# Xinhuan-Imperial/Lattice-Boltzmann-Method-GPU

Measured on NVIDIA B200. Metric: MLUPS, higher is better.
Workload: dtype f64

## Files before the change

### lattice_boltzmann_method_gpu_b200/csrc/lbm_api.cu

```cuda
#include <algorithm>
#include <charconv>
#include <chrono>
#include <cmath>
#include <cstdarg>
#include <cstdio>
#include <cstdlib>
#include <cstring>
#include <deque>
#include <memory>
#include <fstream>
#include <iostream>
#include <new>
#include <sstream>
#include <string>
#include <thread>
#include <vector>

#include "lbm_internal.h"
#include "geo_text.h"
#include "vtk_format.h"

namespace lbm {

static thread_local std::string g_create_error;
// ... 110 lines not shown
    size_t scratch_ints = 0;
    double last_S = 0.0;
    std::vector<long long> plane_first;
    T *d_stage = nullptr;
    size_t stage_elems = 0;
    cudaStream_t st_copy = nullptr;
    cudaEvent_t ev_gathered[2] = {nullptr, nullptr}, ev_copied[2] = {nullptr, nullptr};
    long long pend_i0 = 0, pend_i1 = 0;
    bool interior_pending = false;
    T *peer_buf[2][2] = {{nullptr, nullptr}, {nullptr, nullptr}};
    long long peer_qs[2] = {0, 0}, peer_c0[2] = {0, 0}, peer_own[2] = {0, 0};
    T *d_mail[2] = {nullptr, nullptr}, *peer_mail[2] = {nullptr, nullptr};
    long long mail_ms = 0, mail_G = 0;
    bool mail_live[2] = {false, false};
    T *d_stage_out[2] = {nullptr, nullptr}, *d_stage_in[2] = {nullptr, nullptr};
    bool mail_staged[2] = {false, false};
    unsigned long long *d_sync = nullptr;
    unsigned long long *peer_sync[2] = {nullptr, nullptr};
    int64_t sync_base = 0;
    cudaEvent_t ev_face[2] = {nullptr, nullptr};
    SolverBase *inproc_nb[2] = {nullptr, nullptr};
    bool sparse = false;
    long long n_lo_stored = 0, stored_box = 0;
    long long sp_first = 0;
    long long nseg = 0;
    long long *d_cart = nullptr, *d_chunk_off = nullptr, *d_plane_seg = nullptr;
    uint32_t *d_nodec = nullptr;
    int8_t *d_labelc = nullptr;
    int32_t *d_rec = nullptr, *d_chunk_cnt = nullptr;
    std::vector<long long> seg_plane_start;
    int32_t *d_sid = nullptr;
    uint2 *d_cmeta = nullptr;
    uint32_t *d_rec_links = nullptr;
    int32_t *d_bcslot = nullptr;
    BcLink<T> *d_bclinks = nullptr;
    std::vector<long long> sid_plane_first;
    long long own_id0 = 0, own_id1 = 0;
    long long halo_id0[2] = {0, 0}, halo_n[2] = {0, 0};
    long long face_id0[2] = {0, 0}, face_n[2] = {0, 0};

    ~Solver() override {
        join_writer();
        cudaSetDevice(d.device);
        auto fr = [](void *p) {
            if (p) cudaFree(p);
        };
        fr(d_flag), fr(d_label_ext), fr(d_label), fr(d_index), fr(d_scratch), fr(d_node), fr(d_seg), fr(d_label8);
        fr(d_fa), fr(d_fb == d_fa ? nullptr : d_fb), fr(d_rho), fr(d_ux), fr(d_uy), fr(d_uz), fr(d_plane_in), fr(d_plane_out);
        fr(d_send[0]), fr(d_send[1]), fr(d_recv[0]), fr(d_recv[1]), fr(d_acc), fr(d_cnt);
        fr(d_sid), fr(d_cmeta), fr(d_rec_links), fr(d_bcslot), fr(d_bclinks);
        fr(d_stage), fr(d_wall), fr(d_wallc), fr(d_cart), fr(d_chunk_off), fr(d_nodec), fr(d_labelc), fr(d_rec), fr(d_chunk_cnt), fr(d_plane_seg);
        fr(d_mail[0]), fr(d_mail[1]), fr(d_stage_out[0]), fr(d_stage_out[1]), fr(d_stage_in[0]), fr(d_stage_in[1]);
        fr(d_sync), fr(d_chk_shadow[0]), fr(d_chk_shadow[1]), fr(d_chk_count), fr(d_pulse), fr(d_barrier);
        if (ev0) cudaEventDestroy(ev0);
        if (ev1) cudaEventDestroy(ev1);
        for (auto &e : ev_face)
            if (e) cudaEventDestroy(e);
        for (int k = 0; k < 2; k++) {
            if (ev_gathered[k]) cudaEventDestroy(ev_gathered[k]);
            if (ev_copied[k]) cudaEventDestroy(ev_copied[k]);
        }
        if (st_copy) cudaStreamDestroy(st_copy);
        if (st) cudaStreamDestroy(st);
    }

    int store_all() const { return d.case_rule == LBM_CASE_LDC ? 1 : 0; }

    std::vector<std::pair<void *, size_t>> allocs;
    template <typename U>
    int dalloc(U **p, size_t n) {
        CK(cudaMalloc((void **)p, std::max<size_t>(n, 1) * sizeof(U)));
        dev_bytes += (int64_t)(n * sizeof(U));
        allocs.emplace_back((void *)*p, n * sizeof(U));
        return 0;
    }
    template <typename U>
    void dfree(U **p) {
        if (!*p) return;
        for (auto &a : allocs)
            if (a.first == (void *)*p) {
                dev_bytes -= (int64_t)a.second;
                a = allocs.back();
                allocs.pop_back();
                break;
            }
        cudaFree((void *)*p);
        *p = nullptr;
    }
    void release_geometry_sized() {
        if (d_fb == d_fa) d_fb = nullptr;
        dfree(&d_fa), dfree(&d_fb), dfree(&d_rho), dfree(&d_ux), dfree(&d_uy), dfree(&d_uz);
        for (int sd = 0; sd < 2; sd++) dfree(&d_send[sd]), dfree(&d_recv[sd]);
        dfree(&d_cart), dfree(&d_nodec), dfree(&d_wallc), dfree(&d_labelc), dfree(&d_rec), dfree(&d_chunk_cnt);
        dfree(&d_cmeta), dfree(&d_rec_links), dfree(&d_bcslot), dfree(&d_bclinks);
        dfree(&d_chunk_off), dfree(&d_plane_seg);
        if (d_stage) cudaFree(d_stage), d_stage = nullptr, stage_elems = 0;
        d_cur = d_nxt = nullptr;
        for (int sd = 0; sd < 2; sd++) peer_buf[sd][0] = peer_buf[sd][1] = nullptr;
    }

    int setup() {
        CK(cudaSetDevice(d.device));
        CK(cudaStreamCreateWithFlags(&st, cudaStreamNonBlocking));
        CK(cudaEventCreate(&ev0));
        CK(cudaEventCreate(&ev1));
        for (auto &e : ev_face) CK(cudaEventCreateWithFlags(&e, cudaEventDisableTiming));
// ... 407 lines not shown
            CK(launch_bc_links<T>(d_nodec, d_wallc, d_cart, d_label8, box, bc, d_plane_in, d_plane_out, own_id0, own_id1, d_tot, nullptr,
                                  nullptr, st));
            CK(cudaMemcpyAsync(&total, d_tot, sizeof(int), cudaMemcpyDeviceToHost, st));
            CK(cudaStreamSynchronize(st));
            dfree(&d_bcslot), dfree(&d_bclinks);
            if (dalloc(&d_bcslot, (size_t)std::max<long long>(ns, 1)) || dalloc(&d_bclinks, (size_t)std::max(total, 1))) return LBM_ERR_NOMEM;
            CK(cudaMemsetAsync(d_tot, 0, sizeof(int), st));
            CK(launch_bc_links<T>(d_nodec, d_wallc, d_cart, d_label8, box, bc, d_plane_in, d_plane_out, own_id0, own_id1, d_tot, d_bcslot,
                                  d_bclinks, st));
            launches += 2;
        }
        qstride = (ns + 64 + 31) & ~31LL;
        if (aa && qstride >= (1LL << 31) / 3) FAIL(LBM_ERR_ARG, "slab of %lld nodes is too large for 32-bit element offsets: use more z-slabs", ns);
        if (!d_fa) {
            const size_t fsize = (size_t)qstride * Q + 64;
            if (dalloc(&d_fa, fsize)) return LBM_ERR_NOMEM;
            if (aa) d_fb = d_fa;
            else if (dalloc(&d_fb, fsize)) return LBM_ERR_NOMEM;
            if (dalloc(&d_rho, (size_t)ns) || dalloc(&d_ux, (size_t)ns) || dalloc(&d_uy, (size_t)ns) || dalloc(&d_uz, (size_t)ns))
                return LBM_ERR_NOMEM;
            for (int sd = 0; sd < 2; sd++) {
                const size_t nb = (size_t)std::max(face_n[sd], halo_n[sd]) * 5;
                if (dalloc(&d_send[sd], nb) || dalloc(&d_recv[sd], nb)) return LBM_ERR_NOMEM;
            }
        }
        InitParams<T> ip{};
        ip.fa = d_fa, ip.fb = d_fb, ip.aa = aa ? 1 : 0, ip.qstride = qstride, ip.label = d_label;
        ip.rho = d_rho, ip.ux = d_ux, ip.uy = d_uy, ip.uz = d_uz;
        ip.box = box, ip.case_rule = d.case_rule, ip.u_max = (T)d.u_max;
        for (int i = 0; i < LBM_MAX_BC; i++) ip.bc[i] = bc[i];
        ip.plane_in = d_plane_in, ip.plane_out = d_plane_out, ip.fluid_label = fluid_label;
        CK(launch_init_sparse<T>(ip, d_cart, ns, st));
        launches++;
        CK(cudaStreamSynchronize(st));
        d_cur = d_fa, d_nxt = d_fb;
        steps = 0;
        have_init = true, have_moments = false, in_step = false;
        detach_neighbours();
        return 0;
    }

    bool speculative_pull() const {
        static const char *const force = getenv("LBM_SPECULATIVE");
        return force ? atoi(force) != 0 : (nfluid * 10 >= (int64_t)(own_z1 - own_z0) * box.plane * 9);
    }
    int preload_kernels(bool resid) {
        const bool peers = lo_halo || hi_halo;
        CK(cudaSetDevice(d.device));
        if (d.math == LBM_MATH_STRICT) CK(preload_step_kernels_strict<T>(d.storage, speculative_pull(), peers, resid));
        else CK(preload_step_kernels_fast<T>(d.storage, speculative_pull(), peers, resid));
        return 0;
    }

    StepParams<T> make_params(long long c0, long long c1, double *acc) {
        StepParams<T> p{};
        p.src = d_cur, p.dst = d_nxt, p.qstride = qstride;
        p.node = d_node, p.wall = d_wall, p.seg = d_seg, p.label8 = d_label8;
        p.rho = d_rho, p.ux = d_ux, p.uy = d_uy, p.uz = d_uz;
        p.resid = acc;
        p.box = box, p.c_begin = c0, p.c_end = c1;
        p.pdl = opt_pdl && !lo_halo && !hi_halo && in_place();
        p.fluid_label = fluid_label;
        p.tau = (T)d.tau;
        p.inv_tau = T(1.0) / p.tau;
        p.om1 = T(1.0) - T(1.0) / p.tau;
        double sc = 1.0;
        if (d.pulse_amp != 0.0) sc = 1.0 + d.pulse_amp * std::sin(2.0 * M_PI * (double)steps / d.pulse_period);
        p.pulse_scale = (T)sc;
        for (int i = 0; i < LBM_MAX_BC; i++) p.bc[i] = bc[i];
        p.plane_in = d_plane_in, p.plane_out = d_plane_out;
        p.parity = (int)(steps & 1);
        p.case_rule = d.case_rule;
        p.u_init = (T)d.u_max;
#ifdef LBM_SELFCHECK
        if (chk_prepare() == 0) {
            p.chk_lo[0] = d_fa, p.chk_hi[0] = d_fa + chk_elems, p.chk_lo[1] = d_fb, p.chk_hi[1] = d_fb + chk_elems;
            p.chk_shadow[0] = d_chk_shadow[0], p.chk_shadow[1] = d_fb == d_fa ? d_chk_shadow[0] : d_chk_shadow[1];
            p.chk_count = d_chk_count, p.chk_launch = ++chk_launch_id;
        }
#endif
        p.speculative = speculative_pull();
        return p;
    }
    int launch_range(long long c0, long long c1, bool moments, bool resid, double *acc, int face_sides = 0) {
        if (c1 <= c0) return 0;
        StepParams<T> p = make_params(c0, c1, acc);
        const int which = d_nxt == d_fa ? 0 : 1;
        for (int sd = 0; sd < 2; sd++) {
            if (!(face_sides & (1 << sd)) || !peer_mail[sd]) continue;
            T *dst = peer_mail[sd] + (p.parity ? 5 * mail_ms : 0);
            if (sd == 1) p.peer_up = dst, p.peer_up_qs = mail_ms, p.peer_up_c0 = mail_G, p.peer_up_own = mail_G;
            else p.peer_dn = dst, p.peer_dn_qs = mail_ms, p.peer_dn_c0 = mail_G, p.peer_dn_own = mail_G;
            p.peer_mail = 1, p.face_c0 = c0;
            p.mail[sd] = d_mail[sd], p.mail_ms = mail_ms, p.mail_G = mail_G;
        }
        if ((face_sides & 2) && peer_buf[1][which]) {
            p.peer_up = peer_buf[1][which], p.peer_up_qs = peer_qs[1], p.peer_up_c0 = peer_c0[1], p.peer_up_own = peer_own[1];
            p.face_c0 = sparse ? face_id0[1] : c0;
        }
        if ((face_sides & 1) && peer_buf[0][which]) {
            p.peer_dn = peer_buf[0][which], p.peer_dn_qs = peer_qs[0], p.peer_dn_c0 = peer_c0[0], p.peer_dn_own = peer_own[0];
            p.face_c0 = sparse ? face_id0[0] : c0;
        }
        if (sparse) {
            SparseParams<T> sp{};
            sp.base = p, sp.rec = d_rec, sp.nodec = d_nodec, sp.wallc = d_wallc;
            {
                static const int spw_env = getenv("LBM_SPW") ? atoi(getenv("LBM_SPW")) : 0;
                sp.spw = spw_env > 0 ? spw_env : 1;
            }
            const long long zA = c0 / box.plane - (own_z0 - box.z0), zB = c1 / box.plane - (own_z0 - box.z0);
            sp.seg_begin = seg_plane_start[(size_t)zA], sp.seg_end = seg_plane_start[(size_t)zB];
            if (d.storage == LBM_STORE_SPARSE_AA) {
                sp.cartc = d_cart, sp.cmeta = d_cmeta, sp.rec_links = d_rec_links, sp.bcslot = d_bcslot, sp.bclinks = d_bclinks;
                sp.id_begin = sid_plane_first[(size_t)(c0 / box.plane)], sp.id_end = sid_plane_first[(size_t)(c1 / box.plane)];
                sp.halo_lo_n = (int)halo_n[0], sp.halo_hi0 = (int)halo_id0[1];
                sp.pdl = sp.base.pdl;
                if (sp.base.parity == 0 ? sp.id_end <= sp.id_begin : sp.seg_end <= sp.seg_begin) return 0;
                if (d.math == LBM_MATH_STRICT) CK(launch_step_sparse_aa_strict<T>(sp, moments, resid, st));
                else CK(launch_step_sparse_aa_fast<T>(sp, moments, resid, st));
                launches++;
                return 0;
            }
            if (sp.seg_end <= sp.seg_begin) return 0;
// ... 10 lines not shown
    long long plane_c(int z_global) const { return (long long)(z_global - box.z0) * box.plane; }

    T *d_pulse = nullptr;
    size_t pulse_cap = 0;
    unsigned *d_barrier = nullptr;
    int sm_count = 0;
    static constexpr int PERSIST_MAX_STEPS = 2048, PERSIST_BAR_WORDS = 64 + 32 * 64;
    int opt_persist = -1;
    int opt_pdl = 1;
    bool use_persist() {
        if (d.storage != LBM_STORE_SPARSE_AA || lo_halo || hi_halo) return false;
#ifdef LBM_SELFCHECK
        return false;
#endif
        return opt_persist > 0;
    }
    int persist_steps(int n, bool moments_last, double *S_dev) {
        if (n <= 0) return 0;
        if (!sm_count) {
            cudaDeviceProp prop;
            CK(cudaGetDeviceProperties(&prop, d.device));
            sm_count = prop.multiProcessorCount;
            CK(cudaMalloc((void **)&d_barrier, PERSIST_BAR_WORDS * sizeof(unsigned)));
        }
        const T *pulse_dev = nullptr;
        if (d.pulse_amp != 0.0) {
            std::vector<T> tab((size_t)n);
            for (int k = 0; k < n; k++) tab[(size_t)k] = (T)(1.0 + d.pulse_amp * std::sin(2.0 * M_PI * (double)(steps + k) / d.pulse_period));
            if ((size_t)n > pulse_cap) {
                if (d_pulse) cudaFree(d_pulse), d_pulse = nullptr;
                pulse_cap = (size_t)std::max(n, 256);
                CK(cudaMalloc((void **)&d_pulse, pulse_cap * sizeof(T)));
            }
            CK(cudaMemcpyAsync(d_pulse, tab.data(), (size_t)n * sizeof(T), cudaMemcpyHostToDevice, st));
            CK(cudaStreamSynchronize(st));
            pulse_dev = d_pulse;
        }
        CK(cudaMemsetAsync(d_barrier, 0, PERSIST_BAR_WORDS * sizeof(unsigned), st));
        SparseParams<T> sp{};
        sp.base = make_params(plane_c(own_z0), plane_c(own_z1), nullptr);
        sp.rec = d_rec, sp.nodec = d_nodec, sp.wallc = d_wallc, sp.spw = 1, sp.cartc = d_cart, sp.cmeta = d_cmeta, sp.rec_links = d_rec_links;
        sp.bcslot = d_bcslot, sp.bclinks = d_bclinks;
        sp.seg_begin = seg_plane_start[0], sp.seg_end = seg_plane_start[(size_t)(own_z1 - own_z0)];
        sp.id_begin = own_id0, sp.id_end = own_id1;
        sp.halo_lo_n = 0, sp.halo_hi0 = INT32_MAX;
        const int parity0 = (int)(steps & 1);
        if (d.math == LBM_MATH_STRICT) CK(launch_sparse_aa_persist_strict<T>(sp, n, parity0, moments_last ? 1 : 0, S_dev, pulse_dev, d_barrier, sm_count, st));
        else CK(launch_sparse_aa_persist_fast<T>(sp, n, parity0, moments_last ? 1 : 0, S_dev, pulse_dev, d_barrier, sm_count, st));
        launches++;
        steps += n;
        return 0;
    }

    int step(int n, float *ms) override {
        if (!have_init) FAIL(LBM_ERR_STATE, "step before initialize");
        if (lo_halo || hi_halo) FAIL(LBM_ERR_STATE, "slab handle: use lbm_step_begin / lbm_step_end");
        if (n < 0) FAIL(LBM_ERR_ARG, "negative step count");
        CK(cudaSetDevice(d.device));
        if (ms) CK(cudaEventRecord(ev0, st));
        if (use_persist()) {
            for (int done = 0; done < n; done += PERSIST_MAX_STEPS) {
                const int nb = std::min(PERSIST_MAX_STEPS, n - done);
                int r = persist_steps(nb, done + nb == n, nullptr);
                if (r) return r;
            }
        } else {
            for (int i = 0; i < n; i++) {
                int r = launch_range(plane_c(own_z0), plane_c(own_z1), i == n - 1, false, nullptr);
                if (r) return r;
                std::swap(d_cur, d_nxt);
                steps++;
            }
        }
        if (n > 0) have_moments = true;
        if (ms) {
            CK(cudaEventRecord(ev1, st));
            CK(cudaEventSynchronize(ev1));
            CK(cudaEventElapsedTime(ms, ev0, ev1));
        } else {
            CK(cudaStreamSynchronize(st));
        }
        return 0;
    }

    double *step_acc = nullptr;
    bool step_nosync = false;
    static constexpr unsigned long long SYNC_TIMEOUT_NS = 20ull * 1000000000ull;
    int step_begin(int flags) override { return step_begin_ex(flags, nullptr); }
    int step_begin_ex(int flags, double *acc) {
        if (!have_init) FAIL(LBM_ERR_STATE, "step before initialize");
        if (in_step) FAIL(LBM_ERR_STATE, "lbm_step_begin called twice");
        CK(cudaSetDevice(d.device));
        const bool mom = flags & LBM_STEP_MOMENTS, res = flags & LBM_STEP_VELSUM;
        if (in_place() && ((lo_halo && !peer_buf[0][0] && !peer_mail[0]) || (hi_halo && !peer_buf[1][0] && !peer_mail[1])))
            FAIL(LBM_ERR_STATE, "in-place storage exchanges slab faces by peer stores only: call lbm_p2p_attach first");
        step_flags = flags;
        step_acc = acc ? acc : d_acc, step_nosync = acc != nullptr;
        if (res && !acc) CK(cudaMemsetAsync(d_acc, 0, sizeof(double), st));
        const unsigned long long done = (unsigned long long)(steps - sync_base);
        if (peer_sync[0] || peer_sync[1]) {
            CK(launch_slab_wait(d_sync, peer_sync[0] ? done : 0ull, peer_sync[1] ? done : 0ull, SYNC_TIMEOUT_NS, st));
            launches++;
        }
        for (int sd = 0; sd < 2; sd++)
            if (inproc_nb[sd]) CK(cudaStreamWaitEvent(st, inproc_nb[sd]->face_event((int)((steps + 1) & 1)), 0));
        int r;
        const int zt = own_z1 - 1, zb = own_z0;
        long long i0 = plane_c(own_z0), i1 = plane_c(own_z1);
        if (hi_halo) {
            const int sides = 2 | ((lo_halo && zb == zt) ? 1 : 0);
            if ((r = launch_range(plane_c(zt), plane_c(zt + 1), mom, res, step_acc, sides))) return r;
            if (!fused(1)) {
                if (sparse) CK(launch_halo_pack_sparse<T>(d_nxt, qstride, face_id0[1], face_n[1], 1, d_send[1], face_n[1], st));
                else CK(launch_halo_pack<T>(d_nxt, qstride, box, zt - box.z0, 1, d_send[1], st));
                launches++;
            }
            i1 = plane_c(zt);
        }
        if (lo_halo && !(hi_halo && zb == zt)) {
            if ((r = launch_range(plane_c(zb), plane_c(zb + 1), mom, res, step_acc, 1))) return r;
// ... 1583 lines not shown
```

### lattice_boltzmann_method_gpu_b200/csrc/lbm_internal.h

```cpp
#pragma once
#include <cstdint>
#include <cuda_runtime.h>

#include "../../include/lbm_b200.h"

namespace lbm {

constexpr int Q = 19;
constexpr uint32_t NODE_SKIP = 1u;
constexpr uint32_t NODE_LINKS = 0x7FFFEu;
constexpr uint32_t NODE_WALLS_ONLY = 0x80000000u;
constexpr uint32_t NODE_HAS_BC = 0x40000000u;

enum : uint8_t { SEG_BULK = 0, SEG_MIXED = 1, SEG_EMPTY = 2 };

struct BcEntry {
    int kind, naxis, nsign, vaxis, source, pulsatile;
    double value, init_value;
};

struct Box {
    int nx, ny, nz;
    int px;
    int z0, z1;
// ... 140 lines not shown
template <typename T>
cudaError_t launch_reduce_fields_sparse(const T *ux, const T *uy, const T *uz, const int8_t *labelc, const long long *cart,
                                        Box box, long long i0, long long i1, int kind, int fluid_label, int case_rule,
                                        double *out_dev, cudaStream_t s);
template <typename T>
cudaError_t launch_halo_pack_sparse(const T *f, long long qstride, long long i0, long long n, int side, T *buf,
                                    long long bufstride, cudaStream_t s);
template <typename T>
cudaError_t launch_halo_unpack_sparse(T *f, long long qstride, const int8_t *labelc, int fluid_label, long long i0,
                                      long long n, int side, const T *buf, long long bufstride, cudaStream_t s);

template <typename T>
struct SparseParams {
    StepParams<T> base;
    const int32_t *rec;
    const uint32_t *nodec;
    const uint32_t *wallc;
    long long seg_begin, seg_end;
    int spw;
    const long long *cartc;
    const uint2 *cmeta;
    const uint32_t *rec_links;
    const int32_t *bcslot;
    const BcLink<T> *bclinks;
    long long id_begin, id_end;
    int halo_lo_n, halo_hi0;
    int dk[Q];
    int pdl;
};

template <typename T>
cudaError_t launch_step_sparse_fast(const SparseParams<T> &p, bool moments, bool resid, cudaStream_t s);
template <typename T>
cudaError_t launch_step_sparse_strict(const SparseParams<T> &p, bool moments, bool resid, cudaStream_t s);
template <typename T>
cudaError_t launch_step_sparse_aa_fast(const SparseParams<T> &p, bool moments, bool resid, cudaStream_t s);
template <typename T>
cudaError_t launch_step_sparse_aa_strict(const SparseParams<T> &p, bool moments, bool resid, cudaStream_t s);
template <typename T>
cudaError_t preload_step_kernels_fast(int storage, bool speculative, bool peers, bool resid);
template <typename T>
cudaError_t preload_step_kernels_strict(int storage, bool speculative, bool peers, bool resid);
template <typename T>
cudaError_t launch_sparse_aa_persist_fast(const SparseParams<T> &p, int nsteps, int parity0, int moments_last, double *S,
                                          const T *pulse, unsigned *barrier, int sm_count, cudaStream_t s);
template <typename T>
cudaError_t launch_sparse_aa_persist_strict(const SparseParams<T> &p, int nsteps, int parity0, int moments_last, double *S,
                                            const T *pulse, unsigned *barrier, int sm_count, cudaStream_t s);
template <typename T>
cudaError_t launch_step_dense_fast(const StepParams<T> &p, bool moments, bool resid, int storage, cudaStream_t s);
template <typename T>
cudaError_t launch_step_dense_strict(const StepParams<T> &p, bool moments, bool resid, int storage, cudaStream_t s);

}
```

### lattice_boltzmann_method_gpu_b200/csrc/lbm_step_fast.cu

```cuda
#include "step_dense.cuh"

namespace lbm {
template <typename T>
cudaError_t launch_step_dense_fast(const StepParams<T> &p, bool moments, bool resid, int storage, cudaStream_t s) {
    return launch_step_dense_impl<T, false>(p, moments, resid, storage, s);
}
template cudaError_t launch_step_dense_fast<float>(const StepParams<float> &, bool, bool, int, cudaStream_t);
template cudaError_t launch_step_dense_fast<double>(const StepParams<double> &, bool, bool, int, cudaStream_t);
}

#include "step_sparse.cuh"
namespace lbm {
template <typename T>
cudaError_t launch_step_sparse_fast(const SparseParams<T> &p, bool moments, bool resid, cudaStream_t s) {
    return launch_step_sparse_impl<T, false>(p, moments, resid, s);
}
template cudaError_t launch_step_sparse_fast<float>(const SparseParams<float> &, bool, bool, cudaStream_t);
template cudaError_t launch_step_sparse_fast<double>(const SparseParams<double> &, bool, bool, cudaStream_t);
}

#include "step_sparse_aa.cuh"
namespace lbm {
template <typename T>
cudaError_t launch_step_sparse_aa_fast(const SparseParams<T> &p, bool moments, bool resid, cudaStream_t s) {
    return launch_step_sparse_aa_impl<T, false>(p, moments, resid, s);
}
template cudaError_t launch_step_sparse_aa_fast<float>(const SparseParams<float> &, bool, bool, cudaStream_t);
template cudaError_t launch_step_sparse_aa_fast<double>(const SparseParams<double> &, bool, bool, cudaStream_t);
template <typename T>
cudaError_t launch_sparse_aa_persist_fast(const SparseParams<T> &p, int nsteps, int parity0, int moments_last, double *S,
                                             const T *pulse, unsigned *barrier, int sm_count, cudaStream_t s) {
    PersistArgs<T> a{nsteps, parity0, moments_last, S ? 1 : 0, S, pulse, barrier};
    return launch_sparse_aa_persist_impl<T, false>(p, a, sm_count, s);
}
template cudaError_t launch_sparse_aa_persist_fast<float>(const SparseParams<float> &, int, int, int, double *, const float *,
                                                             unsigned *, int, cudaStream_t);
template cudaError_t launch_sparse_aa_persist_fast<double>(const SparseParams<double> &, int, int, int, double *, const double *,
                                                              unsigned *, int, cudaStream_t);
}

namespace lbm {
template <typename T>
cudaError_t preload_step_kernels_fast(int storage, bool speculative, bool peers, bool resid) {
    if (storage == LBM_STORE_SPARSE_AA) return preload_step_sparse_aa_impl<T, false>(peers, resid);
    if (storage == LBM_STORE_SPARSE_AB) return preload_step_sparse_impl<T, false>(resid);
    return preload_step_dense_impl<T, false>(storage, speculative, resid);
}
template cudaError_t preload_step_kernels_fast<float>(int, bool, bool, bool);
template cudaError_t preload_step_kernels_fast<double>(int, bool, bool, bool);
}
```

### lattice_boltzmann_method_gpu_b200/csrc/lbm_step_strict.cu

```cuda
#include "step_dense.cuh"

namespace lbm {
template <typename T>
cudaError_t launch_step_dense_strict(const StepParams<T> &p, bool moments, bool resid, int storage, cudaStream_t s) {
    return launch_step_dense_impl<T, true>(p, moments, resid, storage, s);
}
template cudaError_t launch_step_dense_strict<float>(const StepParams<float> &, bool, bool, int, cudaStream_t);
template cudaError_t launch_step_dense_strict<double>(const StepParams<double> &, bool, bool, int, cudaStream_t);
}

#include "step_sparse.cuh"
namespace lbm {
template <typename T>
cudaError_t launch_step_sparse_strict(const SparseParams<T> &p, bool moments, bool resid, cudaStream_t s) {
    return launch_step_sparse_impl<T, true>(p, moments, resid, s);
}
template cudaError_t launch_step_sparse_strict<float>(const SparseParams<float> &, bool, bool, cudaStream_t);
template cudaError_t launch_step_sparse_strict<double>(const SparseParams<double> &, bool, bool, cudaStream_t);
}

#include "step_sparse_aa.cuh"
namespace lbm {
template <typename T>
cudaError_t launch_step_sparse_aa_strict(const SparseParams<T> &p, bool moments, bool resid, cudaStream_t s) {
    return launch_step_sparse_aa_impl<T, true>(p, moments, resid, s);
}
template cudaError_t launch_step_sparse_aa_strict<float>(const SparseParams<float> &, bool, bool, cudaStream_t);
template cudaError_t launch_step_sparse_aa_strict<double>(const SparseParams<double> &, bool, bool, cudaStream_t);
template <typename T>
cudaError_t launch_sparse_aa_persist_strict(const SparseParams<T> &p, int nsteps, int parity0, int moments_last, double *S,
                                             const T *pulse, unsigned *barrier, int sm_count, cudaStream_t s) {
    PersistArgs<T> a{nsteps, parity0, moments_last, S ? 1 : 0, S, pulse, barrier};
    return launch_sparse_aa_persist_impl<T, true>(p, a, sm_count, s);
}
template cudaError_t launch_sparse_aa_persist_strict<float>(const SparseParams<float> &, int, int, int, double *, const float *,
                                                             unsigned *, int, cudaStream_t);
template cudaError_t launch_sparse_aa_persist_strict<double>(const SparseParams<double> &, int, int, int, double *, const double *,
                                                              unsigned *, int, cudaStream_t);
}

namespace lbm {
template <typename T>
cudaError_t preload_step_kernels_strict(int storage, bool speculative, bool peers, bool resid) {
    if (storage == LBM_STORE_SPARSE_AA) return preload_step_sparse_aa_impl<T, true>(peers, resid);
    if (storage == LBM_STORE_SPARSE_AB) return preload_step_sparse_impl<T, true>(resid);
    return preload_step_dense_impl<T, true>(storage, speculative, resid);
}
template cudaError_t preload_step_kernels_strict<float>(int, bool, bool, bool);
template cudaError_t preload_step_kernels_strict<double>(int, bool, bool, bool);
}
```

### lattice_boltzmann_method_gpu_b200/csrc/step_dense.cuh

```cuda
#pragma once
#include <cstdlib>
#include "lattice.cuh"
#include "lbm_internal.h"
#include "init_rule.cuh"

namespace lbm {

template <typename T>
__device__ __forceinline__ T ld_stream(const T *p) {
    return __ldg(p);
}

#ifdef LBM_SELFCHECK
template <typename T>
__device__ __noinline__ void chk_touch(const StepParams<T> &p, const T *a, bool track = true) {
    if (!p.chk_count) return;
    for (int b = 0; b < 2; b++)
        if (a >= p.chk_lo[b] && a < p.chk_hi[b]) {
            if (!track) return;
            const unsigned long long tag = ((unsigned long long)p.chk_launch << 32) |
                                           (unsigned long long)((unsigned)blockIdx.x * blockDim.x + threadIdx.x + 1u);
            const unsigned long long old = atomicExch(p.chk_shadow[b] + (a - p.chk_lo[b]), tag);
            if ((old >> 32) == p.chk_launch && old != tag) atomicAdd(p.chk_count + 1, 1ull);
            return;
        }
    atomicAdd(p.chk_count, 1ull);
}
#define LBM_CHK(p_, a_) chk_touch(p_, a_)
#define LBM_CHK_BOUNDS(p_, a_) chk_touch(p_, a_, false)
#else
#define LBM_CHK(p_, a_) ((void)0)
#define LBM_CHK_BOUNDS(p_, a_) ((void)0)
#endif

template <typename T>
__device__ __forceinline__ T bc_speed(const StepParams<T> &p, const BcEntry &e, int gx, int gz, T pulse) {
    T u = bc_speed_unscaled<T>(e, p.box, p.plane_in, p.plane_out, gx, gz);
    if (e.pulsatile) u = u * pulse;
    return u;
}

template <typename T>
__device__ __forceinline__ T feq_bc_axis(T rw, int cs, T u) {
    if (cs > 0) return rw * (T(1.0) + T(3.0) * u + T(3.0) * u * u);
    if (cs < 0) return rw * (T(1.0) - T(3.0) * u + T(3.0) * u * u);
    return rw * (T(1.0) - T(1.5) * u * u);
}

enum { MODE_AB = 0, MODE_AA_EVEN = 1, MODE_AA_ODD = 2 };

template <typename T>
__device__ __noinline__ uint32_t boundary_node(const StepParams<T> &p, long long c, uint32_t rest, int mode, T rho, T ux,
                                               T uy, T uz, const T *g, const T *fpre, T *out, T pulse) {
// ... 176 lines not shown
#pragma unroll
    for (int q = 0; q < Q; q++) {
        if (MODE == MODE_AA_ODD) {
            const bool remote = (czq(q) > 0 && p.peer_up) || (czq(q) < 0 && p.peer_dn);
            if (q == 0 || (!(node & (1u << oppq(q))) && !remote)) {
                LBM_CHK(p, p.store_base[q] + c);
                p.store_base[q][c] = f[q];
            }
        } else {
            LBM_CHK(p, p.store_base[q] + c);
            p.store_base[q][c] = f[q];
        }
    }
    if (MOMENTS) {
        p.rho[c] = rho, p.ux[c] = ux, p.uy[c] = uy, p.uz[c] = uz;
    }
    if (RESID) velsum += (double)(T)sqrt((double)(ux * ux + uy * uy + uz * uz));
    if (p.peer_up || p.peer_dn) push_to_peers<T, MODE>(p, (long long)c - p.face_c0, node, f);
    if (node & NODE_LINKS) {
        const uint32_t wl = (node & NODE_WALLS_ONLY) ? (node & NODE_LINKS)
                                                     : ((WALL_READY || MODE != MODE_AB) ? (wallw & node & NODE_LINKS) : p.wall[c]);
#pragma unroll
        for (int q = 1; q < Q; q++) {
            if (wl & (1u << q)) {
                LBM_CHK(p, p.slot_base[q] + c);
                p.slot_base[q][c] = f[oppq(q)];
            }
        }
        const uint32_t rest = node & NODE_LINKS & ~wl;
        if (rest && (node & NODE_HAS_BC)) {
            T gl[Q], hv[Q];
#pragma unroll
            for (int q = 0; q < Q; q++) gl[q] = f[q];
            if (!keep_pre) {
#pragma unroll
                for (int q = 0; q < Q; q++) fpre[q] = T(0.0);
            }
            const uint32_t wm = boundary_node<T>(p, (long long)c, rest, MODE, rho, ux, uy, uz, gl, fpre, hv, p.pulse_scale);
#pragma unroll
            for (int q = 1; q < Q; q++) {
                if (wm & (1u << q)) {
                    LBM_CHK(p, p.slot_base[q] + c);
                    p.slot_base[q][c] = hv[q];
                }
            }
        }
    }
}

__device__ __forceinline__ void grid_dep_launch() { asm volatile("griddepcontrol.launch_dependents;" ::: "memory"); }
__device__ __forceinline__ void grid_dep_wait() { asm volatile("griddepcontrol.wait;" ::: "memory"); }


template <typename T, bool STRICT, bool MOMENTS, bool RESID, bool SPEC, int CFG, int MODE>
__global__ void __launch_bounds__(cfg_block(CFG), cfg_minb(CFG)) k_step_dense(const __grid_constant__ StepParams<T> p) {
    const Box &b = p.box;
    if (MODE != MODE_AB) grid_dep_launch();
    const long long c = p.c_begin + (long long)blockIdx.x * cfg_block(CFG) + threadIdx.x;
    if (c >= p.c_end) return;
    T f[Q];
    uint32_t node, wallw = 0u;
    const uint32_t kind = p.seg[c >> 5];
    if (SPEC) {
#ifdef LBM_SELFCHECK
        node = p.node[c];
#endif
        if (MODE != MODE_AB) grid_dep_wait();
#pragma unroll
        for (int q = 0; q < Q; q++) {
#ifdef LBM_SELFCHECK
            if (node & NODE_SKIP) LBM_CHK_BOUNDS(p, p.pull_base[q] + c);
            else LBM_CHK(p, p.pull_base[q] + c);
#endif
            f[q] = MODE == MODE_AB ? ld_spec(p.pull_base[q] + c) : ld_spec_rw(p.pull_base[q] + c);
        }
        if (kind == SEG_EMPTY) return;
        node = kind == SEG_MIXED ? p.node[c] : 0u;
        wallw = kind == SEG_MIXED ? p.wall[c] : 0u;
    } else {
        if (kind == SEG_EMPTY) return;
        node = kind == SEG_MIXED ? p.node[c] : 0u;
        wallw = kind == SEG_MIXED ? p.wall[c] : 0u;
        if (MODE != MODE_AB) grid_dep_wait();
    }
    double velsum = 0.0;
    if (!(node & NODE_SKIP)) {
        if (!SPEC) {
#pragma unroll
            for (int q = 0; q < Q; q++) {
                LBM_CHK(p, p.pull_base[q] + c);
                f[q] = MODE == MODE_AB ? ld_stream(p.pull_base[q] + c) : p.pull_base[q][c];
            }
        }
        finish_cell<T, STRICT, MOMENTS, RESID, MODE, true>(p, c, node, wallw, f, velsum);
    }
    if (RESID) {
#pragma unroll
        for (int o = 16; o > 0; o >>= 1) velsum += __shfl_xor_sync(0xffffffffu, velsum, o);
        if ((threadIdx.x & 31) == 0 && velsum != 0.0) atomicAdd(p.resid, velsum);
    }
}

template <typename T, bool STRICT, bool MOMENTS, bool RESID, int CFG, int MODE>
cudaError_t launch_mode(const StepParams<T> &p, cudaStream_t s) {
    constexpr int B = cfg_block(CFG);
    const unsigned nb = (unsigned)((p.c_end - p.c_begin + B - 1) / B);
    cudaLaunchAttribute at[1];
    at[0].id = cudaLaunchAttributeProgrammaticStreamSerialization;
    at[0].val.programmaticStreamSerializationAllowed = 1;
    cudaLaunchConfig_t cfg = {};
    cfg.gridDim = dim3(nb), cfg.blockDim = dim3(B), cfg.dynamicSmemBytes = 0, cfg.stream = s;
    cfg.attrs = at, cfg.numAttrs = (MODE != MODE_AB && p.pdl) ? 1 : 0;
    if (p.speculative) return cudaLaunchKernelEx(&cfg, k_step_dense<T, STRICT, MOMENTS, RESID, true, CFG, MODE>, p);
    return cudaLaunchKernelEx(&cfg, k_step_dense<T, STRICT, MOMENTS, RESID, false, CFG, MODE>, p);
}

template <typename T, bool STRICT, bool MOMENTS, bool RESID>
cudaError_t launch_cfg(const StepParams<T> &p, int storage, cudaStream_t s) {
    constexpr int C = default_cfg<T>();
    if (storage == LBM_STORE_DENSE_AA) {
        if (p.parity == 0) return launch_mode<T, STRICT, MOMENTS, RESID, C, MODE_AA_EVEN>(p, s);
        return launch_mode<T, STRICT, MOMENTS, RESID, C, MODE_AA_ODD>(p, s);
    }
    return launch_mode<T, STRICT, MOMENTS, RESID, C, MODE_AB>(p, s);
}

template <typename T, int MODE>
void set_bases(StepParams<T> &p) {
    for (int q = 0; q < Q; q++) {
        const long long off = (long long)cxq(q) + (long long)p.box.px * cyq(q) + p.box.plane * czq(q);
        p.pull_base[q] = p.src + pull_index<MODE>(q, 0, p.qstride, off);
        p.store_base[q] = p.dst + store_index<MODE>(q, 0, p.qstride, off);
        p.slot_base[q] = p.dst + slot_index<MODE>(q, 0, p.qstride, off);
    }
    for (int side = 0; side < 2; side++) {
        if (!p.mail[side] || MODE == MODE_AB) continue;
        for (int q = 1; q < Q; q++) {
            if (czq(q) != (side == 0 ? 1 : -1)) continue;
            const long long inpl = (long long)cxq(q) + (long long)p.box.px * cyq(q);
            T *A = p.mail[side] + (long long)kslot(q) * p.mail_ms + p.mail_G - p.face_c0;
            T *B = p.mail[side] + (long long)(5 + kslot(q)) * p.mail_ms + p.mail_G - p.face_c0;
            if (MODE == MODE_AA_EVEN) {
                p.pull_base[q] = B;
                p.slot_base[q] = A - inpl;
            } else {
                p.pull_base[q] = A - inpl;
                p.slot_base[q] = B;
            }
        }
    }
}

template <typename T, bool STRICT>
cudaError_t launch_step_dense_impl(const StepParams<T> &p_in, bool moments, bool resid, int storage, cudaStream_t s) {
    if (p_in.c_end <= p_in.c_begin) return cudaSuccess;
    StepParams<T> p = p_in;
    if (storage == LBM_STORE_DENSE_AA) {
        if (p.parity == 0) set_bases<T, MODE_AA_EVEN>(p);
        else set_bases<T, MODE_AA_ODD>(p);
    } else {
        set_bases<T, MODE_AB>(p);
    }
    if (moments && resid) return launch_cfg<T, STRICT, true, true>(p, storage, s);
    if (moments) return launch_cfg<T, STRICT, true, false>(p, storage, s);
    if (resid) return launch_cfg<T, STRICT, false, true>(p, storage, s);
    return launch_cfg<T, STRICT, false, false>(p, storage, s);
}

template <typename K>
inline cudaError_t preload_kernel(K kernel) {
    cudaFuncAttributes a;
    return cudaFuncGetAttributes(&a, kernel);
}
template <typename T, bool STRICT, bool SPEC, int MODE>
cudaError_t preload_dense_mode(bool resid) {
    constexpr int C = default_cfg<T>();
    cudaError_t e;
    if (resid) {
        if ((e = preload_kernel(k_step_dense<T, STRICT, false, true, SPEC, C, MODE>)) != cudaSuccess) return e;
        return preload_kernel(k_step_dense<T, STRICT, true, true, SPEC, C, MODE>);
    }
    if ((e = preload_kernel(k_step_dense<T, STRICT, false, false, SPEC, C, MODE>)) != cudaSuccess) return e;
    return preload_kernel(k_step_dense<T, STRICT, true, false, SPEC, C, MODE>);
}
template <typename T, bool STRICT>
cudaError_t preload_step_dense_impl(int storage, bool speculative, bool resid) {
    cudaError_t e;
    if (storage == LBM_STORE_DENSE_AA) {
        if (speculative) {
            if ((e = preload_dense_mode<T, STRICT, true, MODE_AA_EVEN>(resid)) != cudaSuccess) return e;
            return preload_dense_mode<T, STRICT, true, MODE_AA_ODD>(resid);
        }
        if ((e = preload_dense_mode<T, STRICT, false, MODE_AA_EVEN>(resid)) != cudaSuccess) return e;
        return preload_dense_mode<T, STRICT, false, MODE_AA_ODD>(resid);
    }
    return speculative ? preload_dense_mode<T, STRICT, true, MODE_AB>(resid) : preload_dense_mode<T, STRICT, false, MODE_AB>(resid);
}

}
```

Baseline: 21110.

## Add temporally blocked multi-step dense AA pass with wavefront flag synchronization

Adds a persistent kernel that runs D (default 2) AA-pattern time steps in one launch. Blocks claim work tickets for (z-plane, y-band, step) items in a skewed wavefront and wait on per-band acquire/release flags from neighbouring items of the previous step. The aim is to reuse distributions while they are still in L2 across consecutive steps, so less DRAM traffic is needed when the lattice does not fit in L2. In exchange it adds atomic ticketing, spin-waits and flag memory, and relies on cross-block progress guarantees.

```diff
diff --git a/lattice_boltzmann_method_gpu_b200/csrc/lbm_api.cu b/lattice_boltzmann_method_gpu_b200/csrc/lbm_api.cu
--- a/lattice_boltzmann_method_gpu_b200/csrc/lbm_api.cu
+++ b/lattice_boltzmann_method_gpu_b200/csrc/lbm_api.cu
@@ -186,6 +186,7 @@
         fr(d_stage), fr(d_wall), fr(d_wallc), fr(d_cart), fr(d_chunk_off), fr(d_nodec), fr(d_labelc), fr(d_rec), fr(d_chunk_cnt), fr(d_plane_seg);
         fr(d_mail[0]), fr(d_mail[1]), fr(d_stage_out[0]), fr(d_stage_out[1]), fr(d_stage_in[0]), fr(d_stage_in[1]);
         fr(d_sync), fr(d_chk_shadow[0]), fr(d_chk_shadow[1]), fr(d_chk_count), fr(d_pulse), fr(d_barrier);
+        fr(pass.ticket);
         if (ev0) cudaEventDestroy(ev0);
         if (ev1) cudaEventDestroy(ev1);
         for (auto &e : ev_face)
@@ -699,7 +700,8 @@
         return 0;
     }
 
-    StepParams<T> make_params(long long c0, long long c1, double *acc) {
+    StepParams<T> make_params(long long c0, long long c1, double *acc, int64_t at = -1) {
+        if (at < 0) at = steps;
         StepParams<T> p{};
         p.src = d_cur, p.dst = d_nxt, p.qstride = qstride;
         p.node = d_node, p.wall = d_wall, p.seg = d_seg, p.label8 = d_label8;
@@ -712,11 +714,11 @@
         p.inv_tau = T(1.0) / p.tau;
         p.om1 = T(1.0) - T(1.0) / p.tau;
         double sc = 1.0;
-        if (d.pulse_amp != 0.0) sc = 1.0 + d.pulse_amp * std::sin(2.0 * M_PI * (double)steps / d.pulse_period);
+        if (d.pulse_amp != 0.0) sc = 1.0 + d.pulse_amp * std::sin(2.0 * M_PI * (double)at / d.pulse_period);
         p.pulse_scale = (T)sc;
         for (int i = 0; i < LBM_MAX_BC; i++) p.bc[i] = bc[i];
         p.plane_in = d_plane_in, p.plane_out = d_plane_out;
-        p.parity = (int)(steps & 1);
+        p.parity = (int)(at & 1);
         p.case_rule = d.case_rule;
         p.u_init = (T)d.u_max;
 #ifdef LBM_SELFCHECK
@@ -833,6 +835,43 @@
         return 0;
     }
 
+    PassSync pass{};
+    size_t l2_bytes = 0;
+    bool use_pass() {
+        if (d.storage != LBM_STORE_DENSE_AA || lo_halo || hi_halo) return false;
+#ifdef LBM_SELFCHECK
+        return false;
+#endif
+        if (!l2_bytes) {
+            int v = 0;
+            if (cudaDeviceGetAttribute(&v, cudaDevAttrL2CacheSize, d.device) != cudaSuccess || v <= 0) return false;
+            l2_bytes = (size_t)v;
+        }
+        const size_t fsize = ((size_t)qstride * Q + (size_t)box.plane + box.px + 64) * sizeof(T);
+        return fsize > l2_bytes;
+    }
+    int run_pass(bool moments) {
+        const int D = dense_aa_pass_steps<T>();
+        if (!pass.flags) {
+            const size_t words = (size_t)(box.z1 - box.z0) * box.ny + 1;
+            unsigned long long *w = nullptr;
+            if (dalloc(&w, words)) return LBM_ERR_NOMEM;
+            CK(cudaMemsetAsync(w, 0, words * sizeof(unsigned long long), st));
+            int sms = 0;
+            CK(cudaDeviceGetAttribute(&sms, cudaDevAttrMultiProcessorCount, d.device));
+            pass = PassSync{w + 1, w, 0ull, 0ull, sms};
+        }
+        StepParams<T> p[8];
+        if (D > 8) FAIL(LBM_ERR_STATE, "pass of %d steps", D);
+        for (int k = 0; k < D; k++) p[k] = make_params(plane_c(own_z0), plane_c(own_z1), nullptr, steps + k);
+        const int parity0 = (int)(steps & 1);
+        if (d.math == LBM_MATH_STRICT) CK(launch_dense_aa_pass_strict<T>(p, parity0, moments, pass, st));
+        else CK(launch_dense_aa_pass_fast<T>(p, parity0, moments, pass, st));
+        launches++;
+        steps += D;
+        return 0;
+    }
+
     int step(int n, float *ms) override {
         if (!have_init) FAIL(LBM_ERR_STATE, "step before initialize");
         if (lo_halo || hi_halo) FAIL(LBM_ERR_STATE, "slab handle: use lbm_step_begin / lbm_step_end");
@@ -846,7 +885,15 @@
                 if (r) return r;
             }
         } else {
-            for (int i = 0; i < n; i++) {
+            int i = 0;
+            if (use_pass()) {
+                const int D = dense_aa_pass_steps<T>();
+                for (; i + D <= n; i += D) {
+                    int r = run_pass(i + D == n);
+                    if (r) return r;
+                }
+            }
+            for (; i < n; i++) {
                 int r = launch_range(plane_c(own_z0), plane_c(own_z1), i == n - 1, false, nullptr);
                 if (r) return r;
                 std::swap(d_cur, d_nxt);
diff --git a/lattice_boltzmann_method_gpu_b200/csrc/lbm_internal.h b/lattice_boltzmann_method_gpu_b200/csrc/lbm_internal.h
--- a/lattice_boltzmann_method_gpu_b200/csrc/lbm_internal.h
+++ b/lattice_boltzmann_method_gpu_b200/csrc/lbm_internal.h
@@ -216,4 +216,18 @@
 template <typename T>
 cudaError_t launch_step_dense_strict(const StepParams<T> &p, bool moments, bool resid, int storage, cudaStream_t s);
 
+struct PassSync {
+    unsigned long long *flags;
+    unsigned long long *ticket;
+    unsigned long long ticket0;
+    unsigned long long seq;
+    int sm_count;
+};
+template <typename T>
+int dense_aa_pass_steps();
+template <typename T>
+cudaError_t launch_dense_aa_pass_fast(const StepParams<T> *p, int parity0, bool moments_last, PassSync &sync, cudaStream_t s);
+template <typename T>
+cudaError_t launch_dense_aa_pass_strict(const StepParams<T> *p, int parity0, bool moments_last, PassSync &sync, cudaStream_t s);
+
 }
diff --git a/lattice_boltzmann_method_gpu_b200/csrc/lbm_step_fast.cu b/lattice_boltzmann_method_gpu_b200/csrc/lbm_step_fast.cu
--- a/lattice_boltzmann_method_gpu_b200/csrc/lbm_step_fast.cu
+++ b/lattice_boltzmann_method_gpu_b200/csrc/lbm_step_fast.cu
@@ -7,6 +7,18 @@
 }
 template cudaError_t launch_step_dense_fast<float>(const StepParams<float> &, bool, bool, int, cudaStream_t);
 template cudaError_t launch_step_dense_fast<double>(const StepParams<double> &, bool, bool, int, cudaStream_t);
+template <typename T>
+int dense_aa_pass_steps() {
+    return PassCfg<T>::D;
+}
+template int dense_aa_pass_steps<float>();
+template int dense_aa_pass_steps<double>();
+template <typename T>
+cudaError_t launch_dense_aa_pass_fast(const StepParams<T> *p, int parity0, bool moments_last, PassSync &sync, cudaStream_t s) {
+    return launch_dense_aa_pass_impl<T, false>(p, parity0, moments_last, sync, s);
+}
+template cudaError_t launch_dense_aa_pass_fast<float>(const StepParams<float> *, int, bool, PassSync &, cudaStream_t);
+template cudaError_t launch_dense_aa_pass_fast<double>(const StepParams<double> *, int, bool, PassSync &, cudaStream_t);
 }
 
 #include "step_sparse.cuh"
diff --git a/lattice_boltzmann_method_gpu_b200/csrc/lbm_step_strict.cu b/lattice_boltzmann_method_gpu_b200/csrc/lbm_step_strict.cu
--- a/lattice_boltzmann_method_gpu_b200/csrc/lbm_step_strict.cu
+++ b/lattice_boltzmann_method_gpu_b200/csrc/lbm_step_strict.cu
@@ -7,6 +7,12 @@
 }
 template cudaError_t launch_step_dense_strict<float>(const StepParams<float> &, bool, bool, int, cudaStream_t);
 template cudaError_t launch_step_dense_strict<double>(const StepParams<double> &, bool, bool, int, cudaStream_t);
+template <typename T>
+cudaError_t launch_dense_aa_pass_strict(const StepParams<T> *p, int parity0, bool moments_last, PassSync &sync, cudaStream_t s) {
+    return launch_dense_aa_pass_impl<T, true>(p, parity0, moments_last, sync, s);
+}
+template cudaError_t launch_dense_aa_pass_strict<float>(const StepParams<float> *, int, bool, PassSync &, cudaStream_t);
+template cudaError_t launch_dense_aa_pass_strict<double>(const StepParams<double> *, int, bool, PassSync &, cudaStream_t);
 }
 
 #include "step_sparse.cuh"
diff --git a/lattice_boltzmann_method_gpu_b200/csrc/step_dense.cuh b/lattice_boltzmann_method_gpu_b200/csrc/step_dense.cuh
--- a/lattice_boltzmann_method_gpu_b200/csrc/step_dense.cuh
+++ b/lattice_boltzmann_method_gpu_b200/csrc/step_dense.cuh
@@ -1,4 +1,5 @@
 #pragma once
+#include <algorithm>
 #include <cstdlib>
 #include "lattice.cuh"
 #include "lbm_internal.h"
@@ -281,12 +282,8 @@
 __device__ __forceinline__ void grid_dep_wait() { asm volatile("griddepcontrol.wait;" ::: "memory"); }
 
 
-template <typename T, bool STRICT, bool MOMENTS, bool RESID, bool SPEC, int CFG, int MODE>
-__global__ void __launch_bounds__(cfg_block(CFG), cfg_minb(CFG)) k_step_dense(const __grid_constant__ StepParams<T> p) {
-    const Box &b = p.box;
-    if (MODE != MODE_AB) grid_dep_launch();
-    const long long c = p.c_begin + (long long)blockIdx.x * cfg_block(CFG) + threadIdx.x;
-    if (c >= p.c_end) return;
+template <typename T, bool STRICT, bool MOMENTS, bool RESID, bool SPEC, int MODE, bool PASS>
+__device__ __forceinline__ void step_cell(const StepParams<T> &p, long long c, double &velsum) {
     T f[Q];
     uint32_t node, wallw = 0u;
     const uint32_t kind = p.seg[c >> 5];
@@ -294,7 +291,7 @@
 #ifdef LBM_SELFCHECK
         node = p.node[c];
 #endif
-        if (MODE != MODE_AB) grid_dep_wait();
+        if (MODE != MODE_AB && !PASS) grid_dep_wait();
 #pragma unroll
         for (int q = 0; q < Q; q++) {
 #ifdef LBM_SELFCHECK
@@ -310,19 +307,27 @@
         if (kind == SEG_EMPTY) return;
         node = kind == SEG_MIXED ? p.node[c] : 0u;
         wallw = kind == SEG_MIXED ? p.wall[c] : 0u;
-        if (MODE != MODE_AB) grid_dep_wait();
-    }
-    double velsum = 0.0;
+        if (MODE != MODE_AB && !PASS) grid_dep_wait();
+    }
     if (!(node & NODE_SKIP)) {
         if (!SPEC) {
 #pragma unroll
             for (int q = 0; q < Q; q++) {
                 LBM_CHK(p, p.pull_base[q] + c);
-                f[q] = MODE == MODE_AB ? ld_stream(p.pull_base[q] + c) : p.pull_base[q][c];
+                f[q] = MODE == MODE_AB ? ld_stream(p.pull_base[q] + c) : (PASS ? ld_spec_rw(p.pull_base[q] + c) : p.pull_base[q][c]);
             }
         }
         finish_cell<T, STRICT, MOMENTS, RESID, MODE, true>(p, c, node, wallw, f, velsum);
     }
+}
+
+template <typename T, bool STRICT, bool MOMENTS, bool RESID, bool SPEC, int CFG, int MODE>
+__global__ void __launch_bounds__(cfg_block(CFG), cfg_minb(CFG)) k_step_dense(const __grid_constant__ StepParams<T> p) {
+    if (MODE != MODE_AB) grid_dep_launch();
+    const long long c = p.c_begin + (long long)blockIdx.x * cfg_block(CFG) + threadIdx.x;
+    if (c >= p.c_end) return;
+    double velsum = 0.0;
+    step_cell<T, STRICT, MOMENTS, RESID, SPEC, MODE, false>(p, c, velsum);
     if (RESID) {
 #pragma unroll
         for (int o = 16; o > 0; o >>= 1) velsum += __shfl_xor_sync(0xffffffffu, velsum, o);
@@ -396,6 +401,211 @@
     return launch_cfg<T, STRICT, false, false>(p, storage, s);
 }
 
+#ifndef LBM_PASS_F64_D
+#define LBM_PASS_F64_D 2
+#endif
+#ifndef LBM_PASS_F64_W
+#define LBM_PASS_F64_W 128
+#endif
+#ifndef LBM_PASS_F64_MINB
+#define LBM_PASS_F64_MINB 2
+#endif
+#ifndef LBM_PASS_F32_MINB
+#define LBM_PASS_F32_MINB 5
+#endif
+#ifndef LBM_PASS_F64_R
+#define LBM_PASS_F64_R 1
+#endif
+#ifndef LBM_PASS_BATCH
+#define LBM_PASS_BATCH 1
+#endif
+#ifndef LBM_PASS_F32_D
+#define LBM_PASS_F32_D 2
+#endif
+#ifndef LBM_PASS_F32_W
+#define LBM_PASS_F32_W 256
+#endif
+constexpr int PASS_BATCH = LBM_PASS_BATCH;
+template <typename T>
+struct PassCfg;
+template <>
+struct PassCfg<double> {
+    static constexpr int D = LBM_PASS_F64_D, R = LBM_PASS_F64_R, W = LBM_PASS_F64_W, BLOCK = 256, MINB = LBM_PASS_F64_MINB;
+};
+template <>
+struct PassCfg<float> {
+    static constexpr int D = LBM_PASS_F32_D, R = 1, W = LBM_PASS_F32_W, BLOCK = 256, MINB = LBM_PASS_F32_MINB;
+};
+
+template <typename T>
+struct PassParams {
+    StepParams<T> p[PassCfg<T>::D];
+    unsigned long long *flags;
+    unsigned long long *ticket;
+    unsigned long long ticket0;
+    unsigned long long seq0;
+    int nz, nbands, ntowers;
+    long long nitems;
+    long long nticket;
+};
+
+template <typename T>
+__device__ __forceinline__ int pass_band_lo(int tower, int s) {
+    return max(0, tower * PassCfg<T>::W - s);
+}
+template <typename T>
+__device__ __forceinline__ int pass_band_hi(const PassParams<T> &pp, int tower, int s) {
+    return tower == pp.ntowers - 1 ? pp.nbands : (tower + 1) * PassCfg<T>::W - s;
+}
+
+struct PassItem {
+    long long t;
+    long long next;
+    int left;
+    long long c0, c1;
+    unsigned long long *flag;
+    unsigned long long done;
+    int s, live;
+};
+
+template <typename T, bool STRICT, bool MOMENTS, int MODE>
+__device__ __forceinline__ void pass_cells(const StepParams<T> &p, const PassItem &it) {
+    constexpr int B = PassCfg<T>::BLOCK;
+    double velsum = 0.0;
+    const volatile long long &c1 = it.c1;
+    if (p.speculative) {
+#pragma unroll 1
+        for (long long c = it.c0 + threadIdx.x; c < c1; c += B) step_cell<T, STRICT, MOMENTS, false, true, MODE, true>(p, c, velsum);
+    } else {
+#pragma unroll 1
+        for (long long c = it.c0 + threadIdx.x; c < c1; c += B) step_cell<T, STRICT, MOMENTS, false, false, MODE, true>(p, c, velsum);
+    }
+}
+template <typename T, bool STRICT, int PARITY0, bool MOMENTS_LAST, int S>
+__device__ __forceinline__ void pass_step(const PassParams<T> &pp, const PassItem &it) {
+    constexpr int D = PassCfg<T>::D;
+    if constexpr (S < D) {
+        if (it.s == S) {
+            constexpr int MODE = ((PARITY0 + S) & 1) ? MODE_AA_ODD : MODE_AA_EVEN;
+            pass_cells<T, STRICT, MOMENTS_LAST && S == D - 1, MODE>(pp.p[S], it);
+        } else {
+            pass_step<T, STRICT, PARITY0, MOMENTS_LAST, S + 1>(pp, it);
+        }
+    }
+}
+
+template <typename T>
+__device__ __noinline__ void pass_claim(const PassParams<T> &pp, PassItem &it) {
+    constexpr int D = PassCfg<T>::D, R = PassCfg<T>::R, W = PassCfg<T>::W;
+    constexpr int SHIFT = D * (D - 1) / 2;
+    __syncthreads();
+    if (threadIdx.x == 0) {
+        if (it.left == 0) it.next = (long long)(atomicAdd(pp.ticket, (unsigned long long)PASS_BATCH) - pp.ticket0), it.left = PASS_BATCH;
+        it.t = it.next++, it.left--;
+    }
+    __syncthreads();
+    const long long t = it.t;
+    if (t >= pp.nticket) return;
+    if (t >= pp.nitems) {
+        if (threadIdx.x == 0) it.live = 0;
+        __syncthreads();
+        return;
+    }
+    const long long nw = (long long)pp.nz + 2 * (D - 1);
+    int tower = 0;
+    long long tw = t, per_wave = (long long)D * pp.nbands;
+    if (pp.ntowers > 1) {
+        const long long first = nw * (D * W - SHIFT);
+        if (t >= first) {
+            tower = (int)min((long long)pp.ntowers - 1, 1 + (t - first) / (nw * D * W));
+            tw = t - nw * ((long long)tower * D * W - SHIFT);
+        }
+        per_wave = tower == 0 ? D * W - SHIFT
+                              : (tower == pp.ntowers - 1 ? (long long)D * (pp.nbands - (pp.ntowers - 1) * W) + SHIFT : D * W);
+    }
+    const long long w = tw / per_wave;
+    int r = (int)(tw - w * per_wave), s = 0;
+    for (; s < D - 1; s++) {
+        const int n = pass_band_hi<T>(pp, tower, s) - pass_band_lo<T>(tower, s);
+        if (r < n) break;
+        r -= n;
+    }
+    const int b = pass_band_lo<T>(tower, s) + r;
+    const long long z = w - 2 * s;
+    const bool live = z >= 0 && z < pp.nz;
+    if (live && s > 0 && threadIdx.x < 9) {
+        const int zz = (int)z + (int)threadIdx.x / 3 - 1, bb = b + (int)threadIdx.x % 3 - 1;
+        if (zz >= 0 && zz < pp.nz && bb >= 0 && bb < pp.nbands) {
+            const unsigned long long *f = pp.flags + (long long)zz * pp.nbands + bb, need = pp.seq0 + (unsigned long long)s;
+            unsigned long long v;
+            for (;;) {
+                asm volatile("ld.acquire.gpu.global.u64 %0, [%1];" : "=l"(v) : "l"(f) : "memory");
+                if (v >= need) break;
+                __nanosleep(100);
+            }
+        }
+    }
+    __syncthreads();
+    if (threadIdx.x == 0) {
+        const Box &bx = pp.p[0].box;
+        it.s = s, it.live = live;
+        it.c0 = z * bx.plane + (long long)b * R * bx.px;
+        it.c1 = min(it.c0 + (long long)R * bx.px, (z + 1) * bx.plane);
+        it.flag = live && s < D - 1 ? pp.flags + z * pp.nbands + b : nullptr;
+        it.done = pp.seq0 + (unsigned long long)s + 1ull;
+    }
+    __syncthreads();
+}
+
+template <typename T, bool STRICT, int PARITY0, bool MOMENTS_LAST>
+__global__ void __launch_bounds__(PassCfg<T>::BLOCK, PassCfg<T>::MINB) k_dense_aa_pass(const __grid_constant__ PassParams<T> pp) {
+    static_assert(PassCfg<T>::W >= PassCfg<T>::D, "a tower must keep at least one band at every step of the pass");
+    __shared__ PassItem it;
+    if (threadIdx.x == 0) it.left = 0;
+    for (;;) {
+        pass_claim<T>(pp, it);
+        if (it.t >= pp.nticket) return;
+        if (!it.live) continue;
+        pass_step<T, STRICT, PARITY0, MOMENTS_LAST, 0>(pp, it);
+        __syncthreads();
+        if (threadIdx.x == 0 && it.flag) {
+            __threadfence();
+            asm volatile("st.release.gpu.global.u64 [%0], %1;" ::"l"(it.flag), "l"(it.done) : "memory");
+        }
+    }
+}
+
+template <typename T, bool STRICT>
+cudaError_t launch_dense_aa_pass_impl(const StepParams<T> *p, int parity0, bool moments_last, PassSync &sync, cudaStream_t s) {
+    constexpr int D = PassCfg<T>::D, R = PassCfg<T>::R, W = PassCfg<T>::W, B = PassCfg<T>::BLOCK;
+    PassParams<T> pp{};
+    for (int k = 0; k < D; k++) {
+        pp.p[k] = p[k];
+        if (((parity0 + k) & 1) == 0) set_bases<T, MODE_AA_EVEN>(pp.p[k]);
+        else set_bases<T, MODE_AA_ODD>(pp.p[k]);
+    }
+    const Box &bx = p[0].box;
+    pp.nz = bx.z1 - bx.z0;
+    pp.nbands = (bx.ny + R - 1) / R;
+    pp.ntowers = (pp.nbands + W - 1) / W;
+    pp.nitems = ((long long)pp.nz + 2 * (D - 1)) * D * pp.nbands;
+    pp.nticket = (pp.nitems + PASS_BATCH - 1) / PASS_BATCH * PASS_BATCH;
+    pp.flags = sync.flags, pp.ticket = sync.ticket, pp.ticket0 = sync.ticket0, pp.seq0 = sync.seq;
+    const void *k = parity0 ? (moments_last ? (const void *)k_dense_aa_pass<T, STRICT, 1, true> : (const void *)k_dense_aa_pass<T, STRICT, 1, false>)
+                            : (moments_last ? (const void *)k_dense_aa_pass<T, STRICT, 0, true> : (const void *)k_dense_aa_pass<T, STRICT, 0, false>);
+    int per_sm = 0;
+    cudaError_t e = cudaOccupancyMaxActiveBlocksPerMultiprocessor(&per_sm, k, B, 0);
+    if (e != cudaSuccess) return e;
+    if (per_sm < 1) return cudaErrorLaunchOutOfResources;
+    const long long blocks = std::min<long long>((long long)per_sm * sync.sm_count, pp.nitems);
+    void *args[1] = {(void *)&pp};
+    e = cudaLaunchKernel(k, dim3((unsigned)blocks), dim3(B), args, 0, s);
+    if (e != cudaSuccess) return e;
+    sync.ticket0 += (unsigned long long)(pp.nticket + (long long)PASS_BATCH * blocks);
+    sync.seq += D;
+    return cudaSuccess;
+}
+
 template <typename K>
 inline cudaError_t preload_kernel(K kernel) {
     cudaFuncAttributes a;
@@ -416,6 +626,12 @@
 cudaError_t preload_step_dense_impl(int storage, bool speculative, bool resid) {
     cudaError_t e;
     if (storage == LBM_STORE_DENSE_AA) {
+        if (!resid) {
+            if ((e = preload_kernel(k_dense_aa_pass<T, STRICT, 0, false>)) != cudaSuccess) return e;
+            if ((e = preload_kernel(k_dense_aa_pass<T, STRICT, 0, true>)) != cudaSuccess) return e;
+            if ((e = preload_kernel(k_dense_aa_pass<T, STRICT, 1, false>)) != cudaSuccess) return e;
+            if ((e = preload_kernel(k_dense_aa_pass<T, STRICT, 1, true>)) != cudaSuccess) return e;
+        }
         if (speculative) {
             if ((e = preload_dense_mode<T, STRICT, true, MODE_AA_EVEN>(resid)) != cudaSuccess) return e;
             return preload_dense_mode<T, STRICT, true, MODE_AA_ODD>(resid);
```

After: 20590, median of 6. 0.976x the previous value.
